# sidiso/surfh

Hardware: AMD Instinct MI355X
Metric: CG-iterations/sec (forward+adjoint) on 251x251x4000 cube (higher is better)
Workload: dtype f32 (storage and accumulation; products as 2-piece fp16 splits -- 3 products per fp32 product, 1 on the far tails of the spectral response -- on the 16-bit matrix cores, in the spectral-blur GEMM and in the DFT passes)

## Files before the change

### include/surfh_amd.h

```cpp
#ifndef SURFH_AMD_H
#define SURFH_AMD_H

#include <stdint.h>

#ifdef __cplusplus
extern "C" {
#endif

typedef struct surfh_plan surfh_plan;

typedef struct {
    int32_t wslice_start, wslice_stop;
    int32_t n_pointings;
    int32_t n_slit;
    int32_t n_lambda_out;
    int32_t n_alpha_out;
    int32_t srf;
    int32_t na, nb;
    int32_t alpha0;
    int32_t n_alpha_slit;
    int32_t n_beta_slit;
    const int32_t *slit_beta0;
    const double *slit_weights;
    const int32_t *grid_i0;
// ... 215 lines not shown
                        const float *A, const float *B, float *C);
int surfh_gemm_selftest_ksteps(int64_t near_far[2]);
int surfh_gemm_selftest_ms(double *ms);
int32_t surfh_klist_classify(const float *B, int32_t n, int32_t k, int64_t ldb, int32_t perm_p, int32_t perm_lin,
                             int32_t *records, int64_t capacity);
int surfh_launch_geometry(const char *which, int64_t a, int64_t b, int64_t c, int64_t out[4]);
int surfh_debug_prior_passes(surfh_plan *plan, int32_t T, int32_t na, int32_t nb, int32_t kind, int32_t coupling, const float *x_dev,
                             float *g_dev, const float *p0_dev, const float *p1_dev, double mu_reg, double delta, double *sums);
int surfh_debug_planes_passes(surfh_plan *plan, int32_t L, int32_t na, int32_t nb, int32_t kind, int32_t coupling, const float *x_dev,
                              float *g_dev, const float *p0_dev, const float *p1_dev, const double *mu_reg, const double *delta,
                              double *sums);
int surfh_debug_planes_cg(surfh_plan *plan, const char *which, const int64_t *ext, float *v0, float *v1, float *v2, float *v3,
                          float *v4, float *v5, double mu_reg, int32_t update_r, const double *sc_in, double *sc_out);
int surfh_route_decide(int32_t n_alpha, int32_t n_beta, int32_t n_templates, int64_t lp, int32_t verify, int32_t exact,
                       int32_t has_sotf, uint32_t switches, int32_t scan, int64_t out[8]);
void surfh_debug_alloc_count(int64_t *live, int64_t *total);
void surfh_debug_alloc_fail(int64_t nth);
int surfh_mm_step2(double dBd, double dBm, double mBm, double dg, double mg, double step[2]);

typedef struct surfh_tst surfh_tst;
int surfh_tst_create(int32_t n_alpha, int32_t n_beta, int32_t n_lambda, int32_t n_templates, const double *templates,
                     const int32_t *voxels, int64_t n_voxels, const float *S, int32_t device, surfh_tst **out);
int surfh_tst_destroy(surfh_tst *t);
int surfh_tst_forward(surfh_tst *t, const float *maps, float *cube);
int surfh_tst_adjoint(surfh_tst *t, const float *cube, float *maps);
int surfh_tst_fwadj(surfh_tst *t, const float *maps, float *out);
const char *surfh_tst_last_error(void);

int surfh_shepard(int32_t n_seg, const int64_t *pt_off, const float *pt_alpha, const float *pt_lambda,
                  const float *pt_value, const int32_t *n_alpha, const int32_t *n_lambda, int32_t separable,
// ... 17 lines not shown
```

### surfh_amd/_lib.py

```python
from __future__ import annotations

import ctypes as C
import os

import numpy as np

_HERE = os.path.dirname(os.path.abspath(__file__))
LIB_PATH = os.path.join(_HERE, "libsurfh_amd.so")

c_float_p = C.POINTER(C.c_float)
c_double_p = C.POINTER(C.c_double)
c_int32_p = C.POINTER(C.c_int32)
CG_CALLBACK = C.CFUNCTYPE(C.c_int, C.c_void_p, C.c_int32, c_double_p, c_float_p)
c_uint8_p = C.POINTER(C.c_uint8)
SAMPLE_CALLBACK = C.CFUNCTYPE(C.c_int, C.c_void_p, C.c_int32, C.c_int32, c_double_p, c_float_p)


class ChannelDesc(C.Structure):
    _fields_ = [
        ("wslice_start", C.c_int32), ("wslice_stop", C.c_int32),
        ("n_pointings", C.c_int32), ("n_slit", C.c_int32), ("n_lambda_out", C.c_int32),
        ("n_alpha_out", C.c_int32), ("srf", C.c_int32), ("na", C.c_int32), ("nb", C.c_int32),
        ("alpha0", C.c_int32), ("n_alpha_slit", C.c_int32), ("n_beta_slit", C.c_int32),
        ("slit_beta0", c_int32_p), ("slit_weights", c_double_p),
# ... 18 lines not shown
class ImagerDesc(C.Structure):
    _fields_ = [("n_filters", C.c_int32), ("filters", c_double_p), ("decim", C.c_int32), ("sotf", c_double_p)]


EXPORTS = [
    "surfh_last_error", "surfh_version", "surfh_plan_create", "surfh_plan_destroy", "surfh_isize", "surfh_osize",
    "surfh_stream", "surfh_forward", "surfh_adjoint", "surfh_adjoint_ref", "surfh_fwadj", "surfh_forward_dev",
    "surfh_adjoint_dev", "surfh_adjoint_ref_dev", "surfh_fwadj_dev", "surfh_wct_forward", "surfh_wct_adjoint",
    "surfh_wct_fwadj", "surfh_wct_expsol", "surfh_tst_create", "surfh_tst_destroy", "surfh_tst_forward",
    "surfh_tst_adjoint", "surfh_tst_fwadj", "surfh_tst_last_error", "surfh_cg", "surfh_cg_cb", "surfh_mmmg", "surfh_mmmg_huber", "surfh_huber_prior_dev", "surfh_huber_curv_dev", "surfh_mmmg_huber_vox", "surfh_huber_vox_prior_dev", "surfh_huber_vox_curv_dev", "surfh_mmmg_robust", "surfh_mmmg_robust_vox", "surfh_robust_data_dev", "surfh_robust_curv_dev", "surfh_mmmg_huber_planes", "surfh_huber_planes_prior_dev", "surfh_huber_planes_curv_dev", "surfh_cg_planes", "surfh_mmmg_planes", "surfh_cg_planes_cb", "surfh_mmmg_planes_cb", "surfh_cg_planes_begin_dev", "surfh_cg_planes_step_dev", "surfh_cg_planes_rr", "surfh_maps_to_cube", "surfh_cube_to_maps", "surfh_normal_dev",
    "surfh_prior_add_dev", "surfh_spec_supported", "surfh_spec_size", "surfh_to_spec_dev", "surfh_from_spec_dev", "surfh_forward_spec_dev",
    "surfh_adjoint_spec_dev", "surfh_normal_spec_dev", "surfh_prior_spec_add_dev", "surfh_set_prior", "surfh_set_potential", "surfh_get_potential", "surfh_set_prior_coupling", "surfh_get_prior_coupling", "surfh_set_data_weights", "surfh_set_data_weights_dev", "surfh_has_data_weights", "surfh_set_imager", "surfh_imager_osize", "surfh_imager_forward", "surfh_imager_adjoint", "surfh_imager_forward_dev", "surfh_imager_adjoint_dev", "surfh_imager_fwadj", "surfh_set_imager_data", "surfh_has_imager_term", "surfh_dot_dev", "surfh_cg_step_dev", "surfh_cg_dir_dev", "surfh_cg_iter_dev", "surfh_residual_dev",
    "surfh_randn_dev", "surfh_po_data_dev", "surfh_po_prior_dev", "surfh_po_moments", "surfh_po_rhs", "surfh_cg_sample",
    "surfh_cg_begin_dev", "surfh_cg_iter_nosync_dev", "surfh_cg_xupdate_nosync_dev", "surfh_cg_refresh_nosync_dev", "surfh_cg_trace",
    "surfh_profile_enable", "surfh_profile_filter", "surfh_profile_count", "surfh_profile_get", "surfh_profile_reset", "surfh_debug_copy",
    "surfh_debug_dims", "surfh_gemm_selftest", "surfh_gemm_selftest_ksteps", "surfh_gemm_selftest_ms", "surfh_klist_classify", "surfh_launch_geometry", "surfh_route_decide", "surfh_mm_step2",
    "surfh_debug_alloc_count", "surfh_debug_alloc_fail", "surfh_debug_prior_passes",
    "surfh_mmmg_huber_planes_ex", "surfh_huber_planes_prior_dev_ex", "surfh_huber_planes_curv_dev_ex", "surfh_debug_planes_passes",
    "surfh_debug_planes_cg",
    "surfh_shepard", "surfh_shepard_last_error", "surfh_spectral_median", "surfh_nmf_cd", "surfh_templates_last_error",
    "surfh_set_templates", "surfh_get_templates", "surfh_forward_templates", "surfh_adjoint_templates", "surfh_forward_templates_dev",
    "surfh_adjoint_templates_dev", "surfh_cg_templates", "surfh_cg_templates_cb", "surfh_joint_criterion",
    "surfh_cg_nonneg", "surfh_cg_templates_nonneg", "surfh_nn_project_dev", "surfh_cg_planes_nonneg", "surfh_nn_project_planes_dev",
]

_lib = None


def load():
    global _lib
    if _lib is not None:
# ... 105 lines not shown
    L.surfh_cg_xupdate_nosync_dev.argtypes = [vp, vp, vp, vp, C.c_int64]
    L.surfh_cg_refresh_nosync_dev.argtypes = [vp, vp, vp, vp, vp, C.c_int64]
    L.surfh_cg_trace.argtypes = [vp, c_double_p, C.c_int32]; L.surfh_cg_trace.restype = C.c_int32
    L.surfh_profile_enable.argtypes = [vp, C.c_int32]
    L.surfh_profile_filter.argtypes = [vp, C.c_char_p]
    L.surfh_profile_count.argtypes = [vp]; L.surfh_profile_count.restype = C.c_int32
    L.surfh_profile_get.argtypes = [vp, C.c_int32, C.POINTER(C.c_char_p), C.POINTER(C.c_int64), c_double_p]
    L.surfh_profile_reset.argtypes = [vp]
    L.surfh_debug_copy.argtypes = [vp, C.c_char_p, c_float_p, C.c_int64]; L.surfh_debug_copy.restype = C.c_int64
    L.surfh_debug_dims.argtypes = [vp, C.c_char_p, C.POINTER(C.c_int64)]
    L.surfh_gemm_selftest.argtypes = [C.c_int32] * 5 + [c_float_p, c_float_p, c_float_p]
    L.surfh_gemm_selftest_ksteps.argtypes = [C.POINTER(C.c_int64)]
    L.surfh_gemm_selftest_ms.argtypes = [c_double_p]
    L.surfh_klist_classify.argtypes = [c_float_p, C.c_int32, C.c_int32, C.c_int64, C.c_int32, C.c_int32, C.POINTER(C.c_int32), C.c_int64]
    L.surfh_klist_classify.restype = C.c_int32
    L.surfh_launch_geometry.argtypes = [C.c_char_p, C.c_int64, C.c_int64, C.c_int64, C.POINTER(C.c_int64)]
    L.surfh_route_decide.argtypes = [C.c_int32] * 3 + [C.c_int64] + [C.c_int32] * 3 + [C.c_uint32, C.c_int32, C.POINTER(C.c_int64)]
    L.surfh_mm_step2.argtypes = [C.c_double] * 5 + [c_double_p]
    L.surfh_debug_alloc_count.argtypes = [C.POINTER(C.c_int64), C.POINTER(C.c_int64)]
    L.surfh_debug_alloc_count.restype = None
    L.surfh_debug_alloc_fail.argtypes = [C.c_int64]
    L.surfh_debug_alloc_fail.restype = None
    L.surfh_shepard.argtypes = [C.c_int32, C.POINTER(C.c_int64), vp, vp, vp, c_int32_p, c_int32_p, C.c_int32, vp, vp,
                                c_float_p, c_float_p, C.c_float, C.c_float, C.c_float, C.c_float, vp, vp, C.c_int32, vp,
                                c_float_p]
    L.surfh_shepard_last_error.restype = C.c_char_p
    L.surfh_spectral_median.argtypes = [c_float_p, c_float_p, C.c_int64, C.c_int64, C.c_int32, C.c_int32, C.c_int32]
    L.surfh_nmf_cd.argtypes = [c_float_p, C.c_int64, C.c_int64, C.c_int32, c_int32_p, c_float_p, c_float_p, C.c_int32,
                               C.c_double, c_int32_p, c_double_p, c_double_p, c_double_p, C.c_int32, c_float_p]
    L.surfh_templates_last_error.restype = C.c_char_p
# ... 112 lines not shown
```

### surfh_amd/csrc/dft_h2.h

```cpp
#pragma once
#include <hip/hip_runtime.h>

constexpr int DFT_H2_KT = 8;
constexpr size_t DFT_H2_IMAGE_HALFS = (size_t)2 * 2 * DFT_H2_KT * 128 * 16;

struct DftH2Args {
    int kind = 0;
    const float *src = nullptr;
    long ldb = 0, sB = 0;
    int Kn = 0;
    float *dst = nullptr;
    long ldc = 0, sC = 0;
    float e[4] = {1.f, 0.f, 0.f, 1.f};
    float e_alt[4] = {1.f, 0.f, 0.f, 1.f};
    int Rn = 0, rvalid = 0;
    int KP = 0;
    int N = 0, batch = 1;
    int Nv = 0, NvP = 0;
    const float *mhat = nullptr, *tpl = nullptr;
    int T = 0, LP = 0;
    long PL = 0, KBP = 0;
    int mix_l0 = 0;
    float mhat_self = 1.f, mhat_pair = 1.f;
    int mix_Nb = 0;
    const int *vlist = nullptr;
    int nvalid = 0;
    const int *ktab = nullptr, *rtab = nullptr;
    int tabLP = 0;
};

struct DftH2AdjMix {
    const float *hsrc = nullptr;
    long ldh = 0, sH = 0;
    const float *tpl = nullptr;
    int T = 0, LPt = 0;
    float *mpart = nullptr;
    int nslot = 0;
    int kt0 = 0;
    float out_self = 1.f, out_pair = 1.f;
    int Nb = 0;
    const float *prior_src = nullptr;
    float prior_mu = 0.f;
    const int *vlist = nullptr, *kbstart = nullptr;
// ... 10 lines not shown
```

### surfh_amd/csrc/dft_h2.hip

```cpp
#include "dft_h2.h"
#include "lds_attr.h"
#include "prior_eig.h"
#include <cmath>
#include <cstring>

typedef float f32x16 __attribute__((ext_vector_type(16)));
typedef float f32x2 __attribute__((ext_vector_type(2)));
typedef unsigned u32x2 __attribute__((ext_vector_type(2)));
typedef _Float16 f16x8 __attribute__((ext_vector_type(8)));

#ifndef H2_EXP
#define H2_EXP 0
#endif

namespace {

constexpr int BK = 16, RS = 16;
constexpr int PIECE = 128 * RS;
constexpr int KT = DFT_H2_KT;
constexpr int IMG_HALFS = (int)DFT_H2_IMAGE_HALFS;
constexpr int MIX_ROWS = 256;
constexpr size_t LDS_IMG = (size_t)IMG_HALFS * 2;
constexpr size_t LDS_MIX = (size_t)2 * MIX_ROWS * 2 * sizeof(float4);
#ifndef H2_WAVES
// ... 34 lines not shown
    constexpr int TNW = (KIND == 0) ? 16 : 32;
    constexpr int SRC_T = (KIND == 2) ? 64 : 32, DST_T = (KIND == 1) ? 64 : 32;
    const int var = (KIND == 0) ? (l31 & 1) : 0;
    const int lcol = (KIND == 0) ? (l31 >> 1) : l31;
    const int tilesX = g.N / TNW;
    const unsigned ldb4 = (unsigned)(g.ldb * 4), ldc4 = (unsigned)(g.ldc * 4);
    const unsigned c4 = (unsigned)l31 * (KIND == 2 ? 8u : 4u), d4 = (unsigned)l31 * (KIND == 1 ? 8u : 4u);
    const int nk = g.KP / BK;
    const int kin = g.Kn / 2 + 1;
    float4 *mixbuf = reinterpret_cast<float4 *>(lds + IMG_HALFS);

    {
        uint4 *l4 = reinterpret_cast<uint4 *>(lds);
        for (int i = tid; i < IMG_HALFS / 8; i += NTHREADS) l4[i] = img[i];
    }
    const int s0 = (int)((long)NS * blockIdx.x / gridDim.x), s1 = (int)((long)NS * (blockIdx.x + 1) / gridDim.x);
    int ntw = s1 - s0;
    if (ntw > 0 && (long)NWAVES * (s1 - 1) + wave >= NT) --ntw;

    const float4 *mtab = mixbuf;
    float4 tw = make_float4(0.f, 0.f, 0.f, 0.f);
    int mix_kb = -1;
#define H2_MIXTAB(kb_)                                                                                          \
    {                                                                                                           \
        float4 *mt_ = mixbuf + ((kb_) & 1) * (MIX_ROWS * 2);                                                     \
        const int ne = (g.Kn > g.KP ? g.Kn : g.KP) * 2;                                                         \
        const float msc_ = ((kb_) == 0 || 2 * (kb_) == g.mix_Nb) ? g.mhat_self : g.mhat_pair;                   \
        for (int e_ = tid; e_ < ne; e_ += NTHREADS) {                                                           \
            const int k = e_ >> 1, tp = e_ & 1;           \
            float v[4];                                                                                         \
            _Pragma("unroll") for (int i = 0; i < 4; ++i) {                                                     \
// ... 596 lines not shown
        int cus = 0;
        if (hipDeviceGetAttribute(&cus, hipDeviceAttributeMultiprocessorCount, dev) != hipSuccess) return (int)hipErrorInvalidDevice;
        cus_of[dev] = cus;
    }
    const int tnw = g.kind == 0 ? 16 : 32;
    long NT = (long)(g.N / tnw) * g.batch;
    long NS = (NT + NWAVES - 1) / NWAVES;
    if (NS >= 2147483647L / NWAVES) return (int)hipErrorInvalidValue;
    if ((g.ktab || g.rtab) && (g.tabLP < 128 || g.tabLP % 128)) return (int)hipErrorInvalidValue;
    if (g.vlist) {
        if (NT % NWAVES || g.nvalid < 1 || g.nvalid > NS) return (int)hipErrorInvalidValue;
        NS = g.nvalid;
        NT = NS * NWAVES;
    }
    dim3 grid((unsigned)(NS < cus_of[dev] ? NS : cus_of[dev]));
    const uint4 *im = reinterpret_cast<const uint4 *>(img);
    static unsigned long long d0 = 0, d1 = 0, d2 = 0, d3 = 0;
    if (g.mhat) {
        if (int e = ensure_dynamic_lds(dft_h2_kernel<0, true>, LDS_IMG + LDS_MIX, d3)) return e;
        hipLaunchKernelGGL((dft_h2_kernel<0, true>), grid, dim3(NTHREADS), LDS_IMG + LDS_MIX, stream, g, im, kA, (int)NS, NT);
    } else if (g.kind == 0) {
        if (int e = ensure_dynamic_lds(dft_h2_kernel<0, false>, LDS_IMG, d0)) return e;
        hipLaunchKernelGGL((dft_h2_kernel<0, false>), grid, dim3(NTHREADS), LDS_IMG, stream, g, im, kA, (int)NS, NT);
    } else if (g.kind == 1) {
        if (int e = ensure_dynamic_lds(dft_h2_kernel<1, false>, LDS_IMG, d1)) return e;
        hipLaunchKernelGGL((dft_h2_kernel<1, false>), grid, dim3(NTHREADS), LDS_IMG, stream, g, im, kA, (int)NS, NT);
    } else {
        if (int e = ensure_dynamic_lds(dft_h2_kernel<2, false>, LDS_IMG, d2)) return e;
        hipLaunchKernelGGL((dft_h2_kernel<2, false>), grid, dim3(NTHREADS), LDS_IMG, stream, g, im, kA, (int)NS, NT);
    }
// ... 55 lines not shown
```

### surfh_amd/csrc/plan.hip

```cpp
#include "plan_internal.h"

#include <atomic>

namespace surfh_impl {

namespace {
thread_local std::string g_err;
}

int fail(const char *fmt, ...) {
    char buf[1024];
    va_list ap;
    va_start(ap, fmt);
    vsnprintf(buf, sizeof buf, fmt, ap);
    va_end(ap);
    g_err = buf;
    return 1;
}

namespace {
std::atomic<int64_t> g_alloc_live{0}, g_alloc_total{0}, g_alloc_fail_at{0};
}
int dev_raw_alloc(void **p, size_t bytes) {
    *p = nullptr;
// ... 453 lines not shown
            const long m = ((long)b * k) % Nb;
            const double th = 2.0 * M_PI * (double)m / (double)Nb;
            const double c = std::cos(th) * sb, s = std::sin(th) * sb;
            const double w = (k == 0 || (Nb % 2 == 0 && k == Nb / 2)) ? 1.0 : 2.0;
            Gi[((size_t)0 * KBP + k) * NBP + b] = (float)(w * c);
            Gi[((size_t)1 * KBP + k) * NBP + b] = (float)(-w * s);
            Gf[(size_t)b * (2 * KBP) + 0 * KBP + k] = (float)c;
            Gf[(size_t)b * (2 * KBP) + 1 * KBP + k] = (float)(-s);
            GiT[(size_t)b * (2 * KBP) + 0 * KBP + k] = (float)(w * c);
            GiT[(size_t)b * (2 * KBP) + 1 * KBP + k] = (float)(-w * s);
            GfT[((size_t)0 * KBP + k) * NBP + b] = (float)c;
            GfT[((size_t)1 * KBP + k) * NBP + b] = (float)(-s);
        }
}

int otf_support(surfh_plan *p, const surfh_config *cfg, const Route &r, bool ranges, OtfSupport *found) {
    *found = OTF_NONE;
    if (!r.scan_otf) return 0;
    const bool ct = r.ax_a == AX_CT;
    const int nkb = p->Nb / 2 + 1, nch = (int)(p->LP / 128);
    std::vector<int> bmax(nch, -1), amaxk(nch, -1);
    std::vector<double> km(nkb), kam(p->Na);
    for (int l = 0; l < p->Lown; ++l) {
        if (p->planes[l] < 0) continue;
        std::fill(km.begin(), km.end(), 0.0);
        std::fill(kam.begin(), kam.end(), 0.0);
        double amax = 0.0;
        const double *pl = cfg->sotf + (size_t)p->planes[l] * p->Na * nkb * 2;
        for (int a = 0; a < p->Na; ++a)
            for (int k = 0; k < nkb; ++k) {
                const double re = pl[((size_t)a * nkb + k) * 2], im = pl[((size_t)a * nkb + k) * 2 + 1], m2 = re * re + im * im;
// ... 25 lines not shown
    *found = ranges ? OTF_LISTS_RANGES : OTF_LISTS;
    std::vector<int> tabs((size_t)(ct ? 4 : 3) * nch);
    for (int j = 0; j < nch; ++j) {
        if (ct) {
            const int ja = (std::max(amaxk[j], 0) + p->ctA.R - 1) / p->ctA.R, jb = (std::max(bmax[j], 0) + p->ctB->R - 1) / p->ctB->R;
            tabs[j] = std::min(std::max(ja / 16 + 1, 2), p->ctA.KT);
            tabs[nch + j] = std::min(std::max(jb / 16 + 1, 2), p->ctB->KT);
            tabs[2 * nch + j] = bmax[j];
            tabs[3 * nch + j] = amaxk[j];
            continue;
        }
        tabs[j] = std::min(std::max((amaxk[j] + 16) / 16, 2), p->KPa / 16);
        tabs[nch + j] = std::min(std::max((bmax[j] + 16) / 16, 2), p->KPb / 16);
        tabs[2 * nch + j] = bmax[j] + 1;
    }
    if (ranges && p->otf_tabs.upload(tabs)) return 1;
    return 0;
}

unsigned read_route_switches() {
    static const struct { const char *name; bool dflt; } sw[SW_COUNT] = {
        {"SURFH_DFT_H2", true}, {"SURFH_DFT_CT", true}, {"SURFH_DFT_DENSE", false}, {"SURFH_NO_FUSED_MIX", false},
        {"SURFH_ADJ_FUSED", true}, {"SURFH_OTF_PROD", true}, {"SURFH_OTF_SUPPORT", true}, {"SURFH_OTF_RANGES", true}};
    unsigned m = 0;
    for (int i = 0; i < SW_COUNT; ++i) m |= (unsigned)env_on(sw[i].name, sw[i].dflt) << i;
    return m;
}

}

Route decide_route(const RouteInput &in, OtfSupport scan) {
    Route r;
    auto axis = [&](int n) {
        if (in.on(SW_DFT_H2) && dft_h2_supported(n, n, in.NAP, in.KBP, in.LP)) return AX_H2;
        if (in.on(SW_DFT_CT) && dft_ct_factor(n, nullptr, nullptr)) return AX_CT;
        return AX_DENSE;
    };
    const AxisKernel a = axis(in.Na), b = axis(in.Nb);
    if (in.verify || in.on(SW_DFT_DENSE) || a == AX_DENSE || b == AX_DENSE) return r;
    r.ax_a = a; r.ax_b = b;
// ... 190 lines not shown
            if ((r0.ax_a == AX_H2 && p->MPa != 128) || (r0.ax_b == AX_H2 && p->MPb != 128)) return bail(fail("internal: dft_h2 needs 128-row folded matrices"));
            std::vector<unsigned short> im(3 * DFT_H2_IMAGE_HALFS, 0);
            if (r0.ax_a == AX_H2) p->h2kA[0] = dft_h2_build_image(Cma.data(), Sma.data(), p->MPa, p->KPa, p->KPa, im.data());
            if (r0.ax_b == AX_H2) {
                p->h2kA[1] = dft_h2_build_image(Gc.data(), Gs.data(), p->MPb, p->KPb, p->KPb, im.data() + DFT_H2_IMAGE_HALFS);
                p->h2kA[2] = dft_h2_build_image(Cf.data(), Sf.data(), p->MPb, p->KPb, p->KPb, im.data() + 2 * DFT_H2_IMAGE_HALFS);
            }
            if (p->h2img.upload(im)) return bail(1);
        }
        if (r0.ax_a == AX_CT && dft_ct_plan_create(p->Na, &p->ctA)) return bail(fail("dft_ct plan (n_alpha = %d) failed", p->Na));
        if (r0.ax_b == AX_CT) {
            if (r0.ax_a == AX_CT && p->Nb == p->Na) p->ctB = &p->ctA;
            else if (dft_ct_plan_create(p->Nb, &p->ctB_own)) return bail(fail("dft_ct plan (n_beta = %d) failed", p->Nb));
        }
        OtfSupport found;
        if (otf_support(p, cfg, r0, rin.on(SW_OTF_RANGES), &found)) return bail(1);
        p->route = decide_route(rin, found);
        if (p->route.fused_tail) {
            const size_t npart = dft_h2_adjmix_part_floats(p->LP, p->Nb / 2 + 1, p->otf_nvalid);
            if (!npart) return bail(fail("the fused adjoint tail could not size its partial sums"));
            if (p->adjmix_part.alloc(npart)) return bail(1);
        }
    }
    const size_t nspec = (size_t)2 * p->PL * LP, ncube = (size_t)p->NBP * p->NAP * LP;
    const size_t nycol = (size_t)2 * p->NAP * p->KBP * LP;
    const size_t nmhat = p->T > 0 ? (size_t)p->T * 2 * p->PL : nspec;
    const size_t nmaps = (size_t)std::max(p->T, 1) * p->PLc;
    const size_t nycm = (size_t)std::max(p->T, 1) * 2 * p->NAP * p->KBP;
    if (p->spec.alloc(nspec) || p->ycol.alloc(nycol) || p->cube.alloc(ncube) || p->mhat.alloc(nmhat) || p->maps_pad.alloc(nmaps) ||
        p->ycol_maps.alloc(nycm))
        return bail(1);
// ... 45 lines not shown
                    c.permA = pP;
                }
            }
        }
        if (c.Cpart.zeros((size_t)c.splitK * c.LdetP * c.NP)) return bail(1);
    }
    p->osize = yoff;
    if (p->a_hi <= p->a_lo) { p->a_lo = 0; p->a_hi = p->Na; }
    if (p->b_hi <= p->b_lo) { p->b_lo = 0; p->b_hi = p->Nb; }
    {
        if (!env_on("SURFH_ALPHA_RANGE", true)) { p->a_lo = 0; p->a_hi = p->Na; p->b_lo = 0; p->b_hi = p->Nb; }
        if (ilv && p->a_hi - p->a_lo < p->Na) {
            const size_t nyc = (size_t)2 * p->NAP * p->KBP * p->LP;
            if (p->ycol_adj.zeros(nyc)) return bail(1);
        }
    }
    {
        const long npixrows = (long)p->NBP * p->NAP;
        bool exact_ok = !p->verify;
        if (env_on("SURFH_ADJ_CLEAR", false)) exact_ok = false;
        std::vector<std::vector<uint8_t>> touched(p->ch.size());
        for (size_t ci = 0; ci < p->ch.size(); ++ci) {
            Channel &c = p->ch[ci];
            const std::vector<int64_t> &dst = c.adjT.host_dst;
            touched[ci].assign((size_t)npixrows, 0);
            const int nchunk = (c.nlam / 4 + 255) / 256;
            std::vector<uint32_t> mask(dst.size(), nchunk > 32 ? 0xFFFFFFFFu : 0u);
            std::vector<int2> ranges(dst.size(), make_int2(0, 0));
            for (size_t r = 0; r < dst.size(); ++r) {
                const long pix = (dst[r] - c.ws0a) / p->LP;
// ... 165 lines not shown
```

### surfh_amd/csrc/plan_diag.hip

```cpp
#include "plan_internal.h"
#include "mm_step.h"

extern "C" {

int surfh_profile_enable(surfh_plan *p, int32_t on) {
    if (!p) return fail("null plan");
    p->prof = on != 0;
    return 0;
}
int surfh_profile_filter(surfh_plan *p, const char *prefix) {
    if (!p) return fail("null plan");
    p->prof_filter = prefix ? prefix : "";
    return 0;
}
int32_t surfh_profile_count(surfh_plan *p) {
    if (!p) return -1;
    hipSetDevice(p->dev);
    prof_collect(p);
    return (int32_t)p->acc_names.size();
}
int surfh_profile_get(surfh_plan *p, int32_t i, const char **name, int64_t *launches, double *ms) {
    if (!p || i < 0 || i >= (int32_t)p->acc_names.size()) return fail("bad profile index");
    auto &e = p->acc[p->acc_names[i]];
    *name = p->acc_names[i].c_str();
// ... 49 lines not shown
    } else if (w == "ksteps") {
        for (auto &c : p->ch)
            for (int i = 0; i < 4; ++i) dims[i] += c.ksteps[i];
        for (int i = 0; i < 4; ++i) dims[i] -= 1;
    } else if (w == "groups") {
        dims[0] = dims[1] = 0;
        for (auto &c : p->ch) { dims[0] += c.fwd.g.NG; dims[1] += c.adjT.g.NG; }
    } else if (w == "dft") {
        dims[0] = p->route.ax_a; dims[1] = p->route.ax_b; dims[2] = p->route.interleaved(); dims[3] = p->route.fused_tail;
    } else if (w == "route" || w == "route2") {
        int64_t f[8];
        route_fields(p->route, f);
        for (int i = 0; i < 4; ++i) dims[i] = f[(w == "route2" ? 4 : 0) + i];
    } else if (w == "trim") {
        dims[0] = p->Leff; dims[1] = p->LP; dims[2] = p->Lown;
    } else if (w == "info") {
        dims[0] = p->lo; dims[1] = p->hi; dims[2] = p->Lown; dims[3] = (int64_t)p->segs.size();
    } else {
        return fail("unknown debug buffer '%s'", w.c_str());
    }
    return 0;
}

int surfh_debug_dims(surfh_plan *p, const char *which, int64_t dims[4]) {
    if (!p) return fail("null plan");
    const float *ptr;
    return resolve(p, which, &ptr, dims);
}

int64_t surfh_debug_copy(surfh_plan *p, const char *which, float *out, int64_t cap) {
// ... 12 lines not shown
    return n;
}

int32_t surfh_klist_classify(const float *B, int32_t n, int32_t k, int64_t ldb, int32_t perm_p, int32_t perm_lin, int32_t *records,
                             int64_t capacity) {
    if (!B || !records || n < 1 || k < 32 || k % 32 || ldb < k) return -fail("surfh_klist_classify: bad arguments");
    if (perm_p && ((perm_p != 1 && perm_p != 2 && perm_p != 4 && perm_p != 8) || perm_lin < 1 || perm_lin % (256 / perm_p) || n % perm_lin))
        return -fail("surfh_klist_classify: bad tile shape");
    std::vector<int> kl;
    int stride = 0;
    long nn = 0, nf = 0;
    build_klist(B, n, k, ldb, 0, 0, 1.0 / 256, 1.0 / 1024, &kl, &stride, &nn, &nf, perm_p, perm_lin);
    if ((int64_t)kl.size() > capacity) return -fail("surfh_klist_classify: capacity too small");
    std::memcpy(records, kl.data(), kl.size() * sizeof(int));
    return (int32_t)(kl.size() / (size_t)stride);
}

int surfh_route_decide(int32_t n_alpha, int32_t n_beta, int32_t n_templates, int64_t lp, int32_t verify, int32_t exact, int32_t has_sotf,
                       uint32_t switches, int32_t scan, int64_t out[8]) {
    if (!out || n_alpha < 2 || n_beta < 2 || n_templates < 0 || lp < 128 || lp % 128 || scan < 0 || scan > 2) return fail("surfh_route_decide: bad arguments");
    RouteInput in;
    in.Na = n_alpha; in.Nb = n_beta; in.T = n_templates; in.NAP = pad64(n_alpha); in.KBP = pad64(n_beta / 2 + 1); in.LP = lp;
    in.verify = verify != 0; in.has_sotf = has_sotf != 0; in.exact = exact; in.switches = switches;
    route_fields(decide_route(in, (OtfSupport)scan), out);
    return 0;
}

int surfh_launch_geometry(const char *which, int64_t a, int64_t b, int64_t c, int64_t out[4]) {
    if (!which || !out) return fail("null argument");
    const std::string w(which);
// ... 138 lines not shown
```

### surfh_amd/csrc/plan_internal.h

```cpp
#pragma once

#include <hip/hip_runtime.h>

#include <algorithm>
#include <array>
#include <cfloat>
#include <cmath>
#include <cstdarg>
#include <cstdio>
#include <cstdlib>
#include <cstring>
#include <functional>
#include <map>
#include <string>
#include <vector>

#include "../../include/surfh_amd.h"
#include "dev_buf.h"
#include "dft_h2.h"
#include "dft_ct.h"
#include "gemm_f32.h"
#include "kernels.h"
#include "tplgrad.h"

// ... 62 lines not shown
    DevEll fwd, adjT, adjRef;
    HostEll adjT_host;
    bool has_ref = false;
    bool bsum = false;
    DevBuf<float> wmat;
};

struct ProfRec {
    const char *name;
    hipEvent_t a, b;
};

enum AxisKernel { AX_DENSE = 0, AX_H2 = 1, AX_CT = 2 };
enum OtfSupport { OTF_NONE = 0, OTF_LISTS = 1, OTF_LISTS_RANGES = 2 };
enum RouteSwitch { SW_DFT_H2, SW_DFT_CT, SW_DFT_DENSE, SW_NO_FUSED_MIX, SW_ADJ_FUSED, SW_OTF_PROD, SW_OTF_SUPPORT, SW_OTF_RANGES, SW_COUNT };
struct RouteInput {
    int Na = 0, Nb = 0, T = 0, exact = 0;
    long NAP = 0, KBP = 0, LP = 0;
    bool verify = false, has_sotf = false;
    unsigned switches = 0;
    bool on(RouteSwitch s) const { return (switches >> s & 1u) != 0; }
};
struct Route {
    AxisKernel ax_a = AX_DENSE, ax_b = AX_DENSE;
    bool mix = false;
    bool prod = false;
    bool fused_tail = false;
    bool scan_otf = false;
    OtfSupport support = OTF_NONE;
    bool tpl_spectral = false;
// ... 60 lines not shown
    bool wblur_fp32 = false;
    bool verify = false;
    int prior_kind = 0;
    int pot[3] = {0, 0, 0};
    int coupling = 0;
    Route route;
    DevBuf<unsigned short> h2img;
    DftCtPlan ctA, ctB_own;
    const DftCtPlan *ctB = &ctB_own;
    int a_lo = 0, a_hi = 0, b_lo = 0, b_hi = 0;
    DevBuf<float> ycol_adj;
    DevBuf<float> adjmix_part;
    DevBuf<int> otf_vlist, otf_kbstart;
    int otf_nvalid = 0;
    DevBuf<int> otf_tabs;
    DevBuf<float> ycol_mix;
    int h2kA[3] = {0, 0, 0};
    DevBuf<float> io_x, io_y, io_cube, hth, mhat2;
    DevBuf<float> gcube;
    std::vector<Channel> ch;
    long isize = 0, osize = 0;
    DevBuf<float> dw, dwy;
    int im_F = 0, im_d = 0;
    long im_osize = 0;
    DevBuf<float> im_g, im_xpad, im_xhat, im_zpad, im_zhat, im_io;
    DevBuf<float> im_y, im_w, im_wy;
    double im_mu = 0.0;
    int ycm_planes = 0;
    std::vector<double> tpl_host;
    DevBuf<int> tg_cidx, tg_pidx;
// ... 111 lines not shown
```

### surfh_amd/csrc/plan_ops.hip

```cpp
#include "plan_internal.h"

namespace surfh_impl {

int prior_add(surfh_plan *p, hipStream_t st, const float *d, float *q, int n_img, float mu_reg) {
    return p->prior_kind == 1 ? launch_prior_joint_add(st, d, q, n_img, p->Na, p->Nb, mu_reg) : launch_prior_add(st, d, q, n_img, p->Na, p->Nb, mu_reg);
}

namespace {

int gemm32(surfh_plan *p, hipStream_t st, const GemmArgs &g) { return p->verify ? launch_gemm_f64acc(st, g) : launch_gemm_f32(st, g); }

int rfft2_planes(surfh_plan *p, const float *src, float *dst, int B) {
    GemmArgs g;
    g.A0 = src; g.lda = p->NBP; g.sA = p->PLc;
    g.B0 = p->Gf; g.ldb = 2 * p->KBP; g.sB = 0;
    g.C = p->ycol_maps; g.ldc = 2 * p->KBP; g.sC = (long)p->NAP * 2 * p->KBP;
    g.M = p->NAP; g.N = 2 * p->KBP; g.K = p->NBP; g.batch = B;
    {
        Prof pr(p, "gemm_dft_rows_fwd_maps");
        LAUNCH_OK(gemm32(p, p->stream, g));
    }
    GemmArgs h;
    h.A0 = p->Ff; h.lda = 2 * p->NAP; h.sA = 0;
    h.B0 = p->ycol_maps; h.B1 = p->ycol_maps + p->KBP; h.ksplitB = p->NAP; h.ldb = 2 * p->KBP;
// ... 91 lines not shown
    const OpCall *tail_scaled = nullptr;
};
struct IrfftCall {
    const float *mix = nullptr;
    const ProdOperand *prod = nullptr;
    bool alpha_range_only = false;
};
struct PassShare {
    float *mid = nullptr;
    int a0 = 0, na = 0;
    int Lrun = 0;
    bool lists = false;
    bool ranges = false;
};

int h2_rows_fwd(surfh_plan *p, const float *src, const PassShare &s) {
    const long LP = p->LP;
    DftH2Args g;
    g.kind = 1; g.src = src + (long)s.a0 * LP; g.ldb = p->NAP * LP; g.sB = LP; g.Kn = p->Nb;
    g.dst = s.mid + 2 * (long)s.a0 * LP; g.ldc = 2 * p->NAP * LP; g.sC = 2 * LP; g.e[0] = 1.f; g.e[3] = -1.f; g.rvalid = p->Nb / 2 + 1;
    g.KP = p->KPb; g.N = s.Lrun; g.batch = s.na;
    if (s.ranges) { g.rtab = p->otf_tabs + 2 * (LP / 128); g.tabLP = (int)LP; }
    Prof pr(p, "dft_h2_rows_fwd");
    LAUNCH_OK(launch_dft_h2(p->stream, g, p->h2img + 2 * DFT_H2_IMAGE_HALFS, p->h2kA[2]));
    return 0;
}
int h2_cols_fwd(surfh_plan *p, float *dst, const PassShare &s, const RfftCall &c) {
    const long LP = p->LP;
    DftH2Args h;
    h.kind = 0; h.src = s.mid; h.ldb = 2 * LP; h.sB = 2 * p->NAP * LP; h.Kn = p->Na;
    h.dst = dst; h.ldc = 2 * p->KBP * LP; h.sC = 2 * LP; h.Rn = p->Na; h.rvalid = p->Na / 2 + 1;
    h.KP = p->KPa; h.N = (int)LP; h.batch = p->Nb / 2 + 1;
    h.e[0] = 1.f; h.e[1] = 1.f; h.e[2] = 1.f; h.e[3] = -1.f;
    h.e_alt[0] = 1.f; h.e_alt[1] = -1.f; h.e_alt[2] = 1.f; h.e_alt[3] = 1.f;
    if (!c.tail_out) {
        Prof pr(p, "dft_h2_cols_fwd");
        LAUNCH_OK(launch_dft_h2(p->stream, h, p->h2img, p->h2kA[0]));
// ... 16 lines not shown
    return 0;
}
int h2_cols_inv(surfh_plan *p, const float *src, const PassShare &s, const IrfftCall &c) {
    const long LP = p->LP;
    const int hb = p->Nb / 2 + 1;
    DftH2Args g;
    g.kind = 0; g.src = src; g.ldb = 2 * p->KBP * LP; g.Kn = p->Na;
    g.dst = s.mid; g.ldc = 2 * p->KBP * LP; g.Rn = p->Na; g.rvalid = p->Na / 2 + 1;
    g.KP = p->KPa; g.N = (int)(hb * LP);
    g.e[0] = 1.f; g.e[1] = -1.f; g.e[2] = 1.f; g.e[3] = 1.f;
    g.e_alt[0] = 1.f; g.e_alt[1] = 1.f; g.e_alt[2] = 1.f; g.e_alt[3] = -1.f;
    if (c.mix) { g.mhat = c.mix; g.tpl = p->tpl; g.T = p->T; g.LP = (int)p->LP; g.PL = p->PL; g.KBP = p->KBP; }
    if (c.mix && c.mix != p->mhat) { g.mhat_self = 1.f; g.mhat_pair = 0.70710678118654752f; g.mix_Nb = p->Nb; }
    if (s.lists) { g.vlist = p->otf_vlist; g.nvalid = p->otf_nvalid; }
    if (s.ranges) { g.ktab = p->otf_tabs; g.tabLP = (int)LP; }
    if (s.Lrun < LP) { g.Nv = s.Lrun; g.NvP = (int)LP; }
    Prof pr(p, c.mix ? "dft_h2_cols_inv_mix" : "dft_h2_cols_inv");
    LAUNCH_OK(launch_dft_h2(p->stream, g, p->h2img, p->h2kA[0]));
    return 0;
}
int h2_rows_inv(surfh_plan *p, float *dst, const PassShare &s) {
    const long LP = p->LP;
    DftH2Args h;
    h.kind = 2; h.src = s.mid + (long)s.a0 * 2 * p->KBP * LP; h.ldb = 2 * LP; h.sB = 2 * p->KBP * LP;
    h.dst = dst + (long)s.a0 * LP; h.ldc = p->NAP * LP; h.sC = LP;
    h.e[0] = 1.f; h.e[1] = -1.f; h.e[2] = 1.f; h.e[3] = 1.f; h.Rn = p->Nb; h.rvalid = p->Nb / 2 + 1;
    h.KP = p->KPb; h.N = s.Lrun; h.batch = s.na;
    if (s.ranges) { h.ktab = p->otf_tabs + LP / 128; h.tabLP = (int)LP; }
    Prof pr(p, "dft_h2_rows_inv");
    LAUNCH_OK(launch_dft_h2(p->stream, h, p->h2img + DFT_H2_IMAGE_HALFS, p->h2kA[1]));
    return 0;
}

int ct_rows_fwd(surfh_plan *p, const float *src, const PassShare &s) {
    const long LP = p->LP;
    DftCtArgs g;
    g.R = p->ctB->R; g.M = p->ctB->M; g.loader = DFT_CT_PLAIN; g.epi = DFT_CT_HSEP; g.sgn = -1.f;
    g.scale = (float)(0.5 / std::sqrt((double)p->Nb));
    g.src = src + (long)s.a0 * LP; g.ldb = p->NAP * LP;
    g.dst = s.mid + 2 * (long)s.a0 * LP; g.ldc = 2 * p->NAP * LP;
    g.ncols = (int)(s.na * LP / 2); g.batch = 1;
    if (s.ranges) { g.rtab = p->otf_tabs + 2 * (LP / 128); g.tabLP = (int)(LP / 2); g.tabShift = 6; }
    Prof pr(p, "dft_ct_rows_fwd");
// ... 1022 lines not shown
```

### surfh_amd/models.py

```python
from __future__ import annotations

import ctypes as C
from math import ceil
from typing import List, Optional, Sequence

import numpy as np

from . import _lib, instru
from .geometry import ChannelGeometry
from .linop import LinOp
from . import potentials as _pot
from .weights import DataWeights
from .spectra import TemplateOps
from .nonneg import NonnegOps


def _ptr(t):
    if isinstance(t, int):
        return C.c_void_p(t)
    return C.c_void_p(t.data_ptr())


class Channel(ChannelGeometry):
    device = 0
# ... 491 lines not shown
        _lib.check(self._L.surfh_profile_enable(self._plan, 1 if on else 0))

    def profile_reset(self):
        _lib.check(self._L.surfh_profile_reset(self._plan))

    def profile(self) -> dict:
        n = self._L.surfh_profile_count(self._plan)
        out = {}
        for i in range(n):
            name, cnt, ms = C.c_char_p(), C.c_int64(), C.c_double()
            _lib.check(self._L.surfh_profile_get(self._plan, i, C.byref(name), C.byref(cnt), C.byref(ms)))
            out[name.value.decode()] = (cnt.value, ms.value)
        return out

    def debug_buffer(self, which: str) -> np.ndarray:
        dims = (C.c_int64 * 4)()
        _lib.check(self._L.surfh_debug_dims(self._plan, which.encode(), dims))
        shape = tuple(int(d) for d in dims)
        if which in ("info", "range", "ksteps", "otf", "trim") or which.startswith("xsinfo:"):
            return np.array(shape)
        while len(shape) > 1 and shape[-1] == 1:
            shape = shape[:-1]
        out = np.empty(int(np.prod(shape)), dtype=np.float32)
        n = self._L.surfh_debug_copy(self._plan, which.encode(), _lib.fptr(out), out.size)
        if n < 0:
            raise RuntimeError(self._L.surfh_last_error().decode())
        return out.reshape(shape)
```

Before: 360.6.

## Balance DFT h2 work across CUs using per-tile cost estimates

Adds a cost-weighted partitioner that computes per-block slice boundaries from a simple cost model of each tile (valid columns, k-table lengths). The boundaries are uploaded alongside the OTF tables, and the h2 DFT kernel reads them in place of its uniform count-based split. The aim is to stop a few heavily loaded workgroups from setting the kernel's duration. The cost split is only kept when it lowers the estimated critical path. With the current weights only the fused mix pass actually uses it; the c2r and r2c passes compute statistics but stay on the uniform split.

```diff
diff --git a/include/surfh_amd.h b/include/surfh_amd.h
--- a/include/surfh_amd.h
+++ b/include/surfh_amd.h
@@ -253,6 +253,7 @@
                           float *v4, float *v5, double mu_reg, int32_t update_r, const double *sc_in, double *sc_out);
 int surfh_route_decide(int32_t n_alpha, int32_t n_beta, int32_t n_templates, int64_t lp, int32_t verify, int32_t exact,
                        int32_t has_sotf, uint32_t switches, int32_t scan, int64_t out[8]);
+int surfh_deal_by_cost(const int32_t *cost, int32_t n, int32_t parts, int32_t *bounds);
 void surfh_debug_alloc_count(int64_t *live, int64_t *total);
 void surfh_debug_alloc_fail(int64_t nth);
 int surfh_mm_step2(double dBd, double dBm, double mBm, double dg, double mg, double step[2]);
diff --git a/surfh_amd/_lib.py b/surfh_amd/_lib.py
--- a/surfh_amd/_lib.py
+++ b/surfh_amd/_lib.py
@@ -56,7 +56,7 @@
     "surfh_randn_dev", "surfh_po_data_dev", "surfh_po_prior_dev", "surfh_po_moments", "surfh_po_rhs", "surfh_cg_sample",
     "surfh_cg_begin_dev", "surfh_cg_iter_nosync_dev", "surfh_cg_xupdate_nosync_dev", "surfh_cg_refresh_nosync_dev", "surfh_cg_trace",
     "surfh_profile_enable", "surfh_profile_filter", "surfh_profile_count", "surfh_profile_get", "surfh_profile_reset", "surfh_debug_copy",
-    "surfh_debug_dims", "surfh_gemm_selftest", "surfh_gemm_selftest_ksteps", "surfh_gemm_selftest_ms", "surfh_klist_classify", "surfh_launch_geometry", "surfh_route_decide", "surfh_mm_step2",
+    "surfh_debug_dims", "surfh_gemm_selftest", "surfh_gemm_selftest_ksteps", "surfh_gemm_selftest_ms", "surfh_klist_classify", "surfh_launch_geometry", "surfh_route_decide", "surfh_mm_step2", "surfh_deal_by_cost",
     "surfh_debug_alloc_count", "surfh_debug_alloc_fail", "surfh_debug_prior_passes",
     "surfh_mmmg_huber_planes_ex", "surfh_huber_planes_prior_dev_ex", "surfh_huber_planes_curv_dev_ex", "surfh_debug_planes_passes",
     "surfh_debug_planes_cg",
@@ -192,6 +192,8 @@
     L.surfh_gemm_selftest_ms.argtypes = [c_double_p]
     L.surfh_klist_classify.argtypes = [c_float_p, C.c_int32, C.c_int32, C.c_int64, C.c_int32, C.c_int32, C.POINTER(C.c_int32), C.c_int64]
     L.surfh_klist_classify.restype = C.c_int32
+    L.surfh_deal_by_cost.argtypes = [C.POINTER(C.c_int32), C.c_int32, C.c_int32, C.POINTER(C.c_int32)]
+    L.surfh_deal_by_cost.restype = C.c_int
     L.surfh_launch_geometry.argtypes = [C.c_char_p, C.c_int64, C.c_int64, C.c_int64, C.POINTER(C.c_int64)]
     L.surfh_route_decide.argtypes = [C.c_int32] * 3 + [C.c_int64] + [C.c_int32] * 3 + [C.c_uint32, C.c_int32, C.POINTER(C.c_int64)]
     L.surfh_mm_step2.argtypes = [C.c_double] * 5 + [c_double_p]
diff --git a/surfh_amd/csrc/deal.h b/surfh_amd/csrc/deal.h
--- /dev/null
+++ b/surfh_amd/csrc/deal.h
@@ -0,0 +1,33 @@
+#pragma once
+#include <cstdint>
+
+inline int deal_by_cost(const int *cost, int n, int parts, int *bounds) {
+    if (n < 0 || parts < 1 || !bounds || (n > 0 && !cost)) return 1;
+    int64_t total = 0;
+    for (int i = 0; i < n; ++i) {
+        if (cost[i] < 0) return 1;
+        total += cost[i];
+    }
+    bounds[0] = 0;
+    if (total == 0) {
+        for (int b = 1; b <= parts; ++b) bounds[b] = (int)((int64_t)n * b / parts);
+        return 0;
+    }
+    int i = 0;
+    int64_t pre = 0;
+    for (int b = 1; b <= parts; ++b) {
+        while (i < n && (pre + cost[i]) * parts <= total * b) pre += cost[i++];
+        bounds[b] = i;
+    }
+    return 0;
+}
+
+inline int64_t deal_critical(const int *cost, const int *bounds, int parts) {
+    int64_t crit = 0;
+    for (int b = 0; b < parts; ++b) {
+        int64_t s = 0;
+        for (int i = bounds[b]; i < bounds[b + 1]; ++i) s += cost[i];
+        if (s > crit) crit = s;
+    }
+    return crit;
+}
diff --git a/surfh_amd/csrc/dft_h2.h b/surfh_amd/csrc/dft_h2.h
--- a/surfh_amd/csrc/dft_h2.h
+++ b/surfh_amd/csrc/dft_h2.h
@@ -27,6 +27,8 @@
     int nvalid = 0;
     const int *ktab = nullptr, *rtab = nullptr;
     int tabLP = 0;
+    const int *bounds = nullptr;
+    int nparts = 0, bounds_ns = 0;
 };
 
 struct DftH2AdjMix {
diff --git a/surfh_amd/csrc/dft_h2.hip b/surfh_amd/csrc/dft_h2.hip
--- a/surfh_amd/csrc/dft_h2.hip
+++ b/surfh_amd/csrc/dft_h2.hip
@@ -72,7 +72,8 @@
         uint4 *l4 = reinterpret_cast<uint4 *>(lds);
         for (int i = tid; i < IMG_HALFS / 8; i += NTHREADS) l4[i] = img[i];
     }
-    const int s0 = (int)((long)NS * blockIdx.x / gridDim.x), s1 = (int)((long)NS * (blockIdx.x + 1) / gridDim.x);
+    const int s0 = g.bounds ? g.bounds[blockIdx.x] : (int)((long)NS * blockIdx.x / gridDim.x);
+    const int s1 = g.bounds ? g.bounds[blockIdx.x + 1] : (int)((long)NS * (blockIdx.x + 1) / gridDim.x);
     int ntw = s1 - s0;
     if (ntw > 0 && (long)NWAVES * (s1 - 1) + wave >= NT) --ntw;
 
@@ -699,6 +700,7 @@
         NT = NS * NWAVES;
     }
     dim3 grid((unsigned)(NS < cus_of[dev] ? NS : cus_of[dev]));
+    if (g.bounds && (g.nparts != (int)grid.x || g.bounds_ns != (int)NS)) return (int)hipErrorInvalidValue;
     const uint4 *im = reinterpret_cast<const uint4 *>(img);
     static unsigned long long d0 = 0, d1 = 0, d2 = 0, d3 = 0;
     if (g.mhat) {
diff --git a/surfh_amd/csrc/plan.hip b/surfh_amd/csrc/plan.hip
--- a/surfh_amd/csrc/plan.hip
+++ b/surfh_amd/csrc/plan.hip
@@ -1,4 +1,5 @@
 #include "plan_internal.h"
+#include "deal.h"
 
 #include <atomic>
 
@@ -491,7 +492,51 @@
         }
 }
 
-int otf_support(surfh_plan *p, const surfh_config *cfg, const Route &r, bool ranges, OtfSupport *found) {
+struct DealWeights { int c0, c1, c2; bool use; };
+constexpr DealWeights DEAL_W_MIX = {4, 3, 0, true}, DEAL_W_C2R = {8, 1, 0, false}, DEAL_W_R2C = {20, 0, 3, false};
+
+int deal_ranges(surfh_plan::Deal &d, const std::vector<int> &cost, int parts, std::vector<int> *ranges = nullptr) {
+    const int n = (int)cost.size();
+    std::vector<int> bc(parts + 1), bk(parts + 1);
+    for (int b = 0; b <= parts; ++b) bk[b] = (int)((long)n * b / parts);
+    if (deal_by_cost(cost.data(), n, parts, bc.data())) return fail("deal_by_cost: bad arguments");
+    d.ns = n; d.parts = parts; d.total = 0;
+    for (int c : cost) d.total += c;
+    d.crit_count = deal_critical(cost.data(), bk.data(), parts);
+    d.crit_cost = deal_critical(cost.data(), bc.data(), parts);
+    if (d.crit_cost >= d.crit_count) { bc = bk; d.crit_cost = d.crit_count; }
+    if (ranges) *ranges = bc;
+    return 0;
+}
+
+int deal_mix(surfh_plan *p, const std::vector<int> &vlist, const std::vector<int> &tabs, bool by_cost, std::vector<int> *ranges) {
+    const int nch = (int)(p->LP / 128);
+    std::vector<int> cost(vlist.size());
+    for (size_t i = 0; i < cost.size(); ++i) {
+        const int chunk = vlist[i] % nch;
+        int c = 0;
+        for (int w = 0; w < 8; ++w)
+            c += (p->Leff < p->LP && chunk * 128 + w * 16 >= p->Leff) ? DEAL_W_MIX.c1 * 2 : DEAL_W_MIX.c0 + DEAL_W_MIX.c1 * tabs[chunk];
+        cost[i] = c;
+    }
+    return deal_ranges(p->deal[surfh_plan::DEAL_MIX], cost, (int)std::min<long>((long)cost.size(), p->n_cu), by_cost && DEAL_W_MIX.use ? ranges : nullptr);
+}
+
+int deal_beta(surfh_plan *p) {
+    const int nch = (int)(p->LP / 128), na = p->a_hi - p->a_lo, nkb = p->KPb / 16;
+    const std::vector<int> &tabs = p->otf_tabs_host;
+    const long tilesX = p->Leff / 32, NT = tilesX * na, NS = (NT + 7) / 8;
+    std::vector<int> c2r(NS, 0), r2c(NS, 0);
+    for (long t = 0; t < NT; ++t) {
+        const int chunk = (int)(t % tilesX) / 4;
+        c2r[t / 8] += DEAL_W_C2R.c0 + DEAL_W_C2R.c1 * tabs[nch + chunk];
+        r2c[t / 8] += DEAL_W_R2C.c0 + DEAL_W_R2C.c1 * nkb + DEAL_W_R2C.c2 * ((tabs[2 * nch + chunk] + 31) / 32);
+    }
+    const int parts = (int)std::min<long>(NS, p->n_cu);
+    return deal_ranges(p->deal[surfh_plan::DEAL_C2R], c2r, parts) || deal_ranges(p->deal[surfh_plan::DEAL_R2C], r2c, parts);
+}
+
+int otf_support(surfh_plan *p, const surfh_config *cfg, const Route &r, bool ranges, bool deal_cost, OtfSupport *found) {
     *found = OTF_NONE;
     if (!r.scan_otf) return 0;
     const bool ct = r.ax_a == AX_CT;
@@ -547,6 +592,13 @@
         tabs[nch + j] = std::min(std::max((bmax[j] + 16) / 16, 2), p->KPb / 16);
         tabs[2 * nch + j] = bmax[j] + 1;
     }
+    if (ranges && !ct) {
+        std::vector<int> mix_ranges;
+        if (deal_mix(p, vlist, tabs, deal_cost, &mix_ranges)) return 1;
+        p->otf_tabs_host = tabs;
+        p->deal[surfh_plan::DEAL_MIX].bounds_at = mix_ranges.empty() ? -1 : (long)tabs.size();
+        tabs.insert(tabs.end(), mix_ranges.begin(), mix_ranges.end());
+    }
     if (ranges && p->otf_tabs.upload(tabs)) return 1;
     return 0;
 }
@@ -557,6 +609,8 @@
         {"SURFH_ADJ_FUSED", true}, {"SURFH_OTF_PROD", true}, {"SURFH_OTF_SUPPORT", true}, {"SURFH_OTF_RANGES", true}};
     unsigned m = 0;
     for (int i = 0; i < SW_COUNT; ++i) m |= (unsigned)env_on(sw[i].name, sw[i].dflt) << i;
+    const char *deal = getenv("SURFH_DFT_DEAL");
+    if (!(deal && !strcmp(deal, "count"))) m |= SW_DFT_DEAL_COST;
     return m;
 }
 
@@ -777,7 +831,7 @@
             else if (dft_ct_plan_create(p->Nb, &p->ctB_own)) return bail(fail("dft_ct plan (n_beta = %d) failed", p->Nb));
         }
         OtfSupport found;
-        if (otf_support(p, cfg, r0, rin.on(SW_OTF_RANGES), &found)) return bail(1);
+        if (otf_support(p, cfg, r0, rin.on(SW_OTF_RANGES), (rin.switches & SW_DFT_DEAL_COST) != 0, &found)) return bail(1);
         p->route = decide_route(rin, found);
         if (p->route.fused_tail) {
             const size_t npart = dft_h2_adjmix_part_floats(p->LP, p->Nb / 2 + 1, p->otf_nvalid);
@@ -853,6 +907,7 @@
             const size_t nyc = (size_t)2 * p->NAP * p->KBP * p->LP;
             if (p->ycol_adj.zeros(nyc)) return bail(1);
         }
+        if (p->route.support == OTF_LISTS_RANGES && !p->otf_tabs_host.empty() && deal_beta(p)) return bail(1);
     }
     {
         const long npixrows = (long)p->NBP * p->NAP;
diff --git a/surfh_amd/csrc/plan_diag.hip b/surfh_amd/csrc/plan_diag.hip
--- a/surfh_amd/csrc/plan_diag.hip
+++ b/surfh_amd/csrc/plan_diag.hip
@@ -1,5 +1,6 @@
 #include "plan_internal.h"
 #include "mm_step.h"
+#include "deal.h"
 
 extern "C" {
 
@@ -87,6 +88,9 @@
         for (int i = 0; i < 4; ++i) dims[i] = f[(w == "route2" ? 4 : 0) + i];
     } else if (w == "trim") {
         dims[0] = p->Leff; dims[1] = p->LP; dims[2] = p->Lown;
+    } else if (w == "deal:mix" || w == "deal:c2r" || w == "deal:r2c") {
+        const surfh_plan::Deal &d = p->deal[w == "deal:mix" ? surfh_plan::DEAL_MIX : w == "deal:c2r" ? surfh_plan::DEAL_C2R : surfh_plan::DEAL_R2C];
+        dims[0] = d.crit_count; dims[1] = d.crit_cost; dims[2] = d.total; dims[3] = d.parts;
     } else if (w == "info") {
         dims[0] = p->lo; dims[1] = p->hi; dims[2] = p->Lown; dims[3] = (int64_t)p->segs.size();
     } else {
@@ -129,6 +133,11 @@
     if ((int64_t)kl.size() > capacity) return -fail("surfh_klist_classify: capacity too small");
     std::memcpy(records, kl.data(), kl.size() * sizeof(int));
     return (int32_t)(kl.size() / (size_t)stride);
+}
+
+int surfh_deal_by_cost(const int32_t *cost, int32_t n, int32_t parts, int32_t *bounds) {
+    if (deal_by_cost(cost, n, parts, bounds)) return fail("surfh_deal_by_cost: bad arguments");
+    return 0;
 }
 
 int surfh_route_decide(int32_t n_alpha, int32_t n_beta, int32_t n_templates, int64_t lp, int32_t verify, int32_t exact, int32_t has_sotf,
diff --git a/surfh_amd/csrc/plan_internal.h b/surfh_amd/csrc/plan_internal.h
--- a/surfh_amd/csrc/plan_internal.h
+++ b/surfh_amd/csrc/plan_internal.h
@@ -100,6 +100,7 @@
 enum AxisKernel { AX_DENSE = 0, AX_H2 = 1, AX_CT = 2 };
 enum OtfSupport { OTF_NONE = 0, OTF_LISTS = 1, OTF_LISTS_RANGES = 2 };
 enum RouteSwitch { SW_DFT_H2, SW_DFT_CT, SW_DFT_DENSE, SW_NO_FUSED_MIX, SW_ADJ_FUSED, SW_OTF_PROD, SW_OTF_SUPPORT, SW_OTF_RANGES, SW_COUNT };
+constexpr unsigned SW_DFT_DEAL_COST = 1u << SW_COUNT;
 struct RouteInput {
     int Na = 0, Nb = 0, T = 0, exact = 0;
     long NAP = 0, KBP = 0, LP = 0;
@@ -190,6 +191,14 @@
     DevBuf<int> otf_vlist, otf_kbstart;
     int otf_nvalid = 0;
     DevBuf<int> otf_tabs;
+    std::vector<int> otf_tabs_host;
+    struct Deal {
+        long bounds_at = -1;
+        int ns = 0, parts = 0;
+        int64_t crit_count = 0, crit_cost = 0, total = 0;
+    };
+    enum { DEAL_MIX, DEAL_C2R, DEAL_R2C, DEAL_KINDS };
+    Deal deal[DEAL_KINDS];
     DevBuf<float> ycol_mix;
     int h2kA[3] = {0, 0, 0};
     DevBuf<float> io_x, io_y, io_cube, hth, mhat2;
diff --git a/surfh_amd/csrc/plan_ops.hip b/surfh_amd/csrc/plan_ops.hip
--- a/surfh_amd/csrc/plan_ops.hip
+++ b/surfh_amd/csrc/plan_ops.hip
@@ -129,13 +129,19 @@
     bool ranges = false;
 };
 
+void deal_attach(const surfh_plan *p, int kind, const PassShare &s, DftH2Args &g) {
+    const surfh_plan::Deal &d = p->deal[kind];
+    if (d.bounds_at < 0 || s.Lrun != p->Leff || (kind != surfh_plan::DEAL_MIX && s.na != p->a_hi - p->a_lo)) return;
+    g.bounds = p->otf_tabs + d.bounds_at; g.nparts = d.parts; g.bounds_ns = d.ns;
+}
+
 int h2_rows_fwd(surfh_plan *p, const float *src, const PassShare &s) {
     const long LP = p->LP;
     DftH2Args g;
     g.kind = 1; g.src = src + (long)s.a0 * LP; g.ldb = p->NAP * LP; g.sB = LP; g.Kn = p->Nb;
     g.dst = s.mid + 2 * (long)s.a0 * LP; g.ldc = 2 * p->NAP * LP; g.sC = 2 * LP; g.e[0] = 1.f; g.e[3] = -1.f; g.rvalid = p->Nb / 2 + 1;
     g.KP = p->KPb; g.N = s.Lrun; g.batch = s.na;
-    if (s.ranges) { g.rtab = p->otf_tabs + 2 * (LP / 128); g.tabLP = (int)LP; }
+    if (s.ranges) { g.rtab = p->otf_tabs + 2 * (LP / 128); g.tabLP = (int)LP; deal_attach(p, surfh_plan::DEAL_R2C, s, g); }
     Prof pr(p, "dft_h2_rows_fwd");
     LAUNCH_OK(launch_dft_h2(p->stream, g, p->h2img + 2 * DFT_H2_IMAGE_HALFS, p->h2kA[2]));
     return 0;
@@ -182,6 +188,7 @@
     if (c.mix && c.mix != p->mhat) { g.mhat_self = 1.f; g.mhat_pair = 0.70710678118654752f; g.mix_Nb = p->Nb; }
     if (s.lists) { g.vlist = p->otf_vlist; g.nvalid = p->otf_nvalid; }
     if (s.ranges) { g.ktab = p->otf_tabs; g.tabLP = (int)LP; }
+    if (s.lists && s.ranges) deal_attach(p, surfh_plan::DEAL_MIX, s, g);
     if (s.Lrun < LP) { g.Nv = s.Lrun; g.NvP = (int)LP; }
     Prof pr(p, c.mix ? "dft_h2_cols_inv_mix" : "dft_h2_cols_inv");
     LAUNCH_OK(launch_dft_h2(p->stream, g, p->h2img, p->h2kA[0]));
@@ -194,7 +201,7 @@
     h.dst = dst + (long)s.a0 * LP; h.ldc = p->NAP * LP; h.sC = LP;
     h.e[0] = 1.f; h.e[1] = -1.f; h.e[2] = 1.f; h.e[3] = 1.f; h.Rn = p->Nb; h.rvalid = p->Nb / 2 + 1;
     h.KP = p->KPb; h.N = s.Lrun; h.batch = s.na;
-    if (s.ranges) { h.ktab = p->otf_tabs + LP / 128; h.tabLP = (int)LP; }
+    if (s.ranges) { h.ktab = p->otf_tabs + LP / 128; h.tabLP = (int)LP; deal_attach(p, surfh_plan::DEAL_C2R, s, h); }
     Prof pr(p, "dft_h2_rows_inv");
     LAUNCH_OK(launch_dft_h2(p->stream, h, p->h2img + DFT_H2_IMAGE_HALFS, p->h2kA[1]));
     return 0;
diff --git a/surfh_amd/models.py b/surfh_amd/models.py
--- a/surfh_amd/models.py
+++ b/surfh_amd/models.py
@@ -529,10 +529,12 @@
         return out
 
     def debug_buffer(self, which: str) -> np.ndarray:
+        if which == "deal":
+            return np.stack([self.debug_buffer("deal:" + k) for k in ("mix", "c2r", "r2c")])
         dims = (C.c_int64 * 4)()
         _lib.check(self._L.surfh_debug_dims(self._plan, which.encode(), dims))
         shape = tuple(int(d) for d in dims)
-        if which in ("info", "range", "ksteps", "otf", "trim") or which.startswith("xsinfo:"):
+        if which in ("info", "range", "ksteps", "otf", "trim") or which.startswith(("xsinfo:", "deal:")):
             return np.array(shape)
         while len(shape) > 1 and shape[-1] == 1:
             shape = shape[:-1]
```

Measured after the change: 362.5, median of 5. No clear change (+0.5%).
